# spirit-man/Planetary-LiDAR-Odometry

Hardware: AMD Instinct MI355X
Metric: IMLS-ICP scan-pairs/s (HDL-64 ~120k-pt scan vs 10-scan map, 20 ICP iterations) (higher is better)
Workload: dtype f64; 1 GPU; config B: HDL-64 scan vs 10-scan local map; a step = 4 independent scan pairs as 4 launch sequences in flight; queries=126189, map_points=1262664, solver=LS (trimmed, t=0.02), search_number=20, inputs=resident in HBM, fused_launch=True, launch_groups=4, parallelism=1 GPU, no process group

## Files before the change

### planetary-lidar-odometry_amd/csrc/project.hip

```cpp
#include <algorithm>
#include <cfloat>

#include "internal.h"
#include "geom.h"

#if defined(__has_builtin) && __has_builtin(__builtin_amdgcn_writelane)
__device__ __forceinline__ int imls_amdgcn_writelane(int v, int sel, int old) {
    return __builtin_amdgcn_writelane(v, sel, old);
}
#else
__device__ int imls_amdgcn_writelane(int v, int sel, int old) __asm("llvm.amdgcn.writelane");
#endif

namespace imlsgpu {
namespace {

constexpr double kInfD = __builtin_huge_val();
constexpr float kInfF = __builtin_huge_valf();
constexpr int kWaveBlock = 256;
typedef float kf4v __attribute__((ext_vector_type(4)));
typedef __attribute__((address_space(4))) const kf4v kconst_f4;
__device__ __forceinline__ int ld_const(const int* p) { return *(const __attribute__((address_space(4))) int*)p; }
__device__ __forceinline__ double ld_const(const double* p) { return *(const __attribute__((address_space(4))) double*)p; }
constexpr int kFallbackBlocks = 64;
// ... 66 lines not shown
    double dot = ns[0] * n0;
    dot = dot + ns[1] * n1;
    dot = dot + ns[2] * n2;
    double a = ns[0] * ns[0];
    a = a + ns[1] * ns[1];
    a = a + ns[2] * ns[2];
    double b = n0 * n0;
    b = b + n1 * n1;
    b = b + n2 * n2;
    const double s = sqrt(a) * sqrt(b);
    if (dot > (cthr + 2e-9) * s) return false;
    if (dot < (cthr - 2e-9) * s && dot >= -s * (1.0 - 1e-12)) return true;
    const double ca = dot / s;
    if (ca > cthr + 1e-9) return false;
    if (ca < cthr - 1e-9 && ca >= -1.0) return true;
    const double angle = acos(ca) * 180.0 / M_PI;
    return angle > thr;
}

template <int KL>
__device__ __forceinline__ void insert_top(float (&lk)[KL], int (&lp)[KL], float d, int pos) {
    bool c[KL];
#pragma unroll
    for (int k = 0; k < KL - 1; ++k) c[k] = d < lk[k];
    c[KL - 1] = true;
#pragma unroll
    for (int k = KL - 1; k >= 1; --k) {
        lp[k] = c[k - 1] ? lp[k - 1] : (c[k] ? pos : lp[k]);
        lk[k] = __builtin_amdgcn_fmed3f(lk[k - 1], d, lk[k]);
    }
    lp[0] = c[0] ? pos : lp[0];
    lk[0] = c[0] ? d : lk[0];
}

__device__ __forceinline__ float fmin_nn(float a, float b) { return a < b ? a : b; }

__device__ __forceinline__ void pin_loaded(const float4& v) { asm volatile("" ::"v"(v.x), "v"(v.y), "v"(v.z)); }

template <int KL>
__device__ __forceinline__ void insert_key(float (&lk)[KL], float d) {
#pragma unroll
    for (int k = KL - 1; k >= 1; --k) lk[k] = __builtin_amdgcn_fmed3f(lk[k - 1], d, lk[k]);
    lk[0] = fmin_nn(d, lk[0]);
}

template <int CAP, bool LAZY_D = false>
__device__ int finish_query(const float xf[3], const double ns[3], const double (&ld)[CAP], const int (&lpos)[CAP],
                            int first, int cnt, double d1, int p1, const TreeView& t, const KParams& kp, float yf[3],
                            float nf[3], int& kq, int qi) {
    if (p1 < 0) return IMLS_REJ_TOO_FAR;
    if (d1 > kp.h2) return IMLS_REJ_TOO_FAR;
    double nn[3];
    if (kp.tv) {
        const double4 v = t.tvn[qi];
        if (v.w == 0.0) return IMLS_REJ_NO_NORMAL;
        nn[0] = v.x; nn[1] = v.y; nn[2] = v.z;
    } else {
        if (!kp.get_normals) return IMLS_REJ_INVALID_NORMAL;
        const float4 n4 = t.mnr[p1];
        nn[0] = n4.x; nn[1] = n4.y; nn[2] = n4.z;
    }
    if (!(isfinite(nn[0]) && isfinite(nn[1]) && isfinite(nn[2]))) return IMLS_REJ_INVALID_NORMAL;
    if (kp.angle_on && angle_reject(ns, nn[0], nn[1], nn[2], kp.angle_thr_deg, kp.cos_thr)) return IMLS_REJ_NORMAL_CONSTRAINT;
    const double xd[3] = {xf[0], xf[1], xf[2]};
    unsigned long long acc = 0ull;
    int nacc = 0;
    constexpr int kChunk = 8;
#pragma unroll
    for (int j0 = 0; j0 < CAP; j0 += kChunk) {
        float4 qn[kChunk];
#pragma unroll
        for (int u = 0; u < kChunk; ++u) {
            const int j = j0 + u;
            const bool inl = j < CAP && j >= first && j < first + cnt;
            qn[u] = t.mnr[inl ? lpos[j < CAP ? j : 0] : p1];
        }
#pragma unroll
        for (int u = 0; u < kChunk; ++u) {
            const int j = j0 + u;
            const bool inl = j < CAP && j >= first && j < first + cnt;
            if (inl) {
                ++kq;
                bool ok = kp.get_normals && isfinite(qn[u].x) && isfinite(qn[u].y) && isfinite(qn[u].z);
                if (ok && kp.angle_on) ok = !angle_reject(ns, qn[u].x, qn[u].y, qn[u].z, kp.angle_thr_deg, kp.cos_thr);
                if (ok) { acc |= 1ull << j; ++nacc; }
            }
        }
    }
    if (nacc < 3) return IMLS_REJ_MLS_FAIL;
    const int target = first + nacc - 1;
    constexpr int kIChunk = IMLS_IMLS_CHUNK;
    float4 qp[kIChunk], qn[kIChunk];
    auto load_chunk = [&](int j0) {
#pragma unroll
        for (int u = 0; u < kIChunk; ++u) {
            const int j = j0 + u;
            const int pj = (j < CAP && (acc & (1ull << j))) ? lpos[j < CAP ? j : 0] : p1;
            qp[u] = t.mpt[pj];
            qn[u] = t.mnr[pj];
        }
    };
    auto pin_chunk = [&]() {
#pragma unroll
        for (int u = 0; u < kIChunk; ++u) {
            pin_loaded(qp[u]);
            pin_loaded(qn[u]);
        }
    };
    double dsel = 0.0;
    if (LAZY_D) {
        int ptg = p1;
#pragma unroll
        for (int j = 0; j < CAP; ++j) ptg = (j == target) ? lpos[j] : ptg;
        const float4 q = t.mpt[ptg];
        load_chunk(0);
        pin_loaded(q);
        pin_chunk();
        dsel = exact_d2(xd, q.x, q.y, q.z);
    } else {
#pragma unroll
        for (int j = 0; j < CAP; ++j) dsel = (j == target) ? ld[j] : dsel;
        load_chunk(0);
        pin_chunk();
    }
    const double hmax = sqrt(dsel) / 3;
    const double ih2 = 1.0 / (hmax * hmax);
    double wsum = 0.0, psum = 0.0;
#pragma unroll
    for (int j0 = 0; j0 < CAP; j0 += kIChunk) {
        if (j0 > 0) {
            if (!__ballot((acc >> j0) != 0ull)) break;
            if (!__ballot((acc >> j0) & ((1ull << kIChunk) - 1ull))) continue;
            load_chunk(j0);
            pin_chunk();
        }
#pragma unroll
        for (int u = 0; u < kIChunk; ++u) {
            const int j = j0 + u;
            if (j >= CAP) break;
            const bool a = (acc >> j) & 1ull;
            if (!__ballot(a)) continue;
            const double dx = xd[0] - (double)qp[u].x, dy = xd[1] - (double)qp[u].y, dz = xd[2] - (double)qp[u].z;
            double dn = dx * dx;
            dn = dn + dy * dy;
            dn = dn + dz * dz;
            const double w = exp(-dn * ih2);
            double pr = (w * dx) * (double)qn[u].x;
            pr = pr + (w * dy) * (double)qn[u].y;
            pr = pr + (w * dz) * (double)qn[u].z;
            wsum += a ? w : 0.0;
            psum += a ? pr : 0.0;
        }
    }
    const double height = psum / (wsum + 1e-5);
    if (isnan(height) || isinf(height)) return IMLS_REJ_NAN_INF_HEIGHT;
    yf[0] = (float)(xd[0] - height * nn[0]);
    yf[1] = (float)(xd[1] - height * nn[1]);
    yf[2] = (float)(xd[2] - height * nn[2]);
    nf[0] = (float)nn[0]; nf[1] = (float)nn[1]; nf[2] = (float)nn[2];
    return -1;
}

__device__ int finish_plane(const float xf[3], const double ns[3], int p1, const TreeView& t, const KParams& kp,
                            float yf[3], float nf[3]) {
    if (p1 < 0) return kp.proj ? IMLS_REJ_TOO_FAR : IMLS_REJ_NO_NORMAL;
    const float4 n4 = t.mnr[p1];
    const double nn[3] = {n4.x, n4.y, n4.z};
    if (!(isfinite(nn[0]) && isfinite(nn[1]) && isfinite(nn[2]))) return IMLS_REJ_INVALID_NORMAL;
    if (kp.angle_on && angle_reject(ns, nn[0], nn[1], nn[2], kp.angle_thr_deg, kp.cos_thr)) return IMLS_REJ_NORMAL_CONSTRAINT;
    const float4 q = t.mpt[p1];
    const double xd[3] = {xf[0], xf[1], xf[2]};
    const double v0 = xd[0] - (double)q.x, v1 = xd[1] - (double)q.y, v2 = xd[2] - (double)q.z;
    double pd = v0 * nn[0];
    pd = pd + v1 * nn[1];
    pd = pd + v2 * nn[2];
    yf[0] = (float)(xd[0] - pd * nn[0]);
    yf[1] = (float)(xd[1] - pd * nn[1]);
    yf[2] = (float)(xd[2] - pd * nn[2]);
    nf[0] = (float)nn[0]; nf[1] = (float)nn[1]; nf[2] = (float)nn[2];
    return -1;
}

__device__ __forceinline__ void plane_row(const float xf[3], const float yf[3], const float nf[3], double a[6], double& b) {
    const double s0 = xf[0], s1 = xf[1], s2 = xf[2];
    const double d0 = yf[0], d1 = yf[1], d2 = yf[2];
    const double n0 = nf[0], n1 = nf[1], n2 = nf[2];
    a[0] = n2 * s1 - n1 * s2;
    a[1] = n0 * s2 - n2 * s0;
    a[2] = n1 * s0 - n0 * s1;
    a[3] = n0; a[4] = n1; a[5] = n2;
    b = n0 * (d0 - s0);
    b = b + n1 * (d1 - s1);
    b = b + n2 * (d2 - s2);
}

template <int NT>
__device__ void block_normeq(const double a[6], double b, double one, double (*red)[kNormEq], double* out) {
    const int lane = threadIdx.x & 63, wv = threadIdx.x >> 6;
    int k = 0;
#pragma unroll
    for (int r = 0; r < 6; ++r) {
#pragma unroll
        for (int c = r; c < 6; ++c) {
            const double v = wave_total(a[r] * a[c]);
            if (lane == 63) red[wv][k] = v;
            ++k;
        }
    }
#pragma unroll
    for (int r = 0; r < 6; ++r) {
        const double v = wave_total(a[r] * b);
        if (lane == 63) red[wv][21 + r] = v;
    }
    {
        const double v = wave_total(one);
        if (lane == 63) red[wv][27] = v;
    }
    __syncthreads();
    if (threadIdx.x < kNormEq) {
        double s = 0.0;
#pragma unroll
        for (int w = 0; w < NT / 64; ++w) s += red[w][threadIdx.x];
        out[threadIdx.x] = s;
    }
    __syncthreads();
}

__device__ __forceinline__ void store_result(int i, int cat, const float xf[3], const float yf[3], const float nf[3],
                                             float4* cs, float4* cd, float4* cn) {
    cs[i] = make_float4(xf[0], xf[1], xf[2], cat == -1 ? 1.f : 0.f);
    if (cat == -1) {
        cd[i] = make_float4(yf[0], yf[1], yf[2], 0.f);
        cn[i] = make_float4(nf[0], nf[1], nf[2], 0.f);
    }
}

#ifdef IMLS_DEBUG_WAVE_TRACE
constexpr int kDbgWaves = 8192;
__device__ unsigned g_dbg_wave[kDbgWaves][16];
#endif


__device__ __forceinline__ bool verlet_skip(float4 xr, float nr, const float xf[3], float r2s, float& w_out,
                                            float& w_low) {
    const float dx = xf[0] - xr.x, dy = xf[1] - xr.y, dz = xf[2] - xr.z;
    const float D = sqrtf(__builtin_fmaf(dx, dx, __builtin_fmaf(dy, dy, dz * dz))) * (1.0f + 1e-6f) + 1e-6f;
    const float g = sqrtf(xr.w) * (1.0f - 1e-6f) - D;
    w_low = g > 0.f ? fminf(g * g, r2s) : -1.0f;
    if (!(g > 0.f) || !(nr < kInfF)) return false;
    const float u = sqrtf(nr) * (1.0f + 1e-6f) + D;
    const float w = fminf(g * g, r2s);
    w_out = w;
    return u * u * (1.0f + 1e-5f) < w;
}

template <int KL>
__device__ __forceinline__ float need_key(const float (&lk)[KL], float r2, int K) {
    const float r2f = r2 * (1.0f + 1e-6f);
    int cnt_r = 0;
    float dK = kInfF, d1 = kInfF;
#pragma unroll
    for (int j = 0; j < KL; ++j) {
        const bool in = lk[j] <= r2f;
        cnt_r += in ? 1 : 0;
        if (in && d1 == kInfF && lk[j] > 1e-15f) d1 = lk[j];
        if (j == K - 1) dK = lk[j];
    }
    return cnt_r >= K ? fmaxf(dK, d1) : (IMLS_UNDER_SKIN > 0 ? r2f : kInfF);
}

template <int KL>
struct IdKeys {
    static constexpr unsigned IDM = KL <= 32 ? 31u : 63u;
    static constexpr unsigned kSentinel = 0x7F7FFFFFu & ~IDM;
    __device__ static __forceinline__ float lo(float k) { return __uint_as_float(__float_as_uint(k) & ~IDM); }
    __device__ static __forceinline__ float hi(float k) { return __uint_as_float(__float_as_uint(k) | IDM); }
    __device__ static __forceinline__ unsigned id(float k) { return __float_as_uint(k) & IDM; }
    __device__ static __forceinline__ float make(float d, unsigned s) { return __uint_as_float((__float_as_uint(d) & ~IDM) | s); }
    __device__ static __forceinline__ float empty(unsigned s) { return __uint_as_float(kSentinel | s); }
    __device__ static __forceinline__ bool real(float k) { return (__float_as_uint(k) & ~IDM) < kSentinel; }
};

template <int KL>
__device__ __forceinline__ float need_key_ids(const float (&lk)[KL], float r2, int K) {
    using I = IdKeys<KL>;
    const float r2f = r2 * (1.0f + 1e-6f);
    int cnt_r = 0;
    float dK = kInfF, d1 = kInfF;
#pragma unroll
    for (int j = 0; j < KL; ++j) {
        const float up = I::hi(lk[j]);
        const bool in = I::real(lk[j]) && up <= r2f;
        cnt_r += in ? 1 : 0;
        if (in && d1 == kInfF && I::lo(lk[j]) > 1e-15f) d1 = up;
        if (j == K - 1) dK = up;
    }
    return cnt_r >= K ? fmaxf(dK, d1) : (IMLS_UNDER_SKIN > 0 ? r2f : kInfF);
}

#ifndef IMLS_KNN_WAVES
#define IMLS_KNN_WAVES 5
#endif
#define IMLS_KNN_ATTR __attribute__((amdgpu_waves_per_eu(KL <= 26 ? IMLS_KNN_WAVES : 2)))
template <int KL>
__device__ __forceinline__ void knn_wave_body(TreeView t, const float4* __restrict__ spt,
                                                         const unsigned* __restrict__ qperm, int N,
                                                         const double* __restrict__ pose,
                                                         const int* __restrict__ done, KParams kp,
                                                         const double* __restrict__ delta,
                                                         int* __restrict__ lists, float* __restrict__ wlist,
                                                         float4* __restrict__ xref, float* __restrict__ nref,
                                                         int use_prev, unsigned long long* __restrict__ nbr_stats,
                                                         int bx) {
    if (done && ld_const(done)) return;
    __shared__ int snode[kWaveBlock / 64][kWaveStack];
    __shared__ float4 sboxa[kWaveBlock / 64][kWaveStack];
    __shared__ float2 sboxb[kWaveBlock / 64][kWaveStack];
    __shared__ int spos[KL][kWaveBlock];
    const int tid = threadIdx.x, lane = tid & 63;
    int* const mypos = &spos[0][tid];
    using IK = IdKeys<KL>;
    const int wv = __builtin_amdgcn_readfirstlane(tid >> 6);
    const int qp = kp.packet;
    const int slot = (bx * (kWaveBlock / 64) + wv) * qp + lane;
    const bool active = lane < qp && slot < N;
    float xf[3] = {0.f, 0.f, 0.f};
    float w_prev = 0.f, n_prev = 0.f;
    float4 x_prev = make_float4(0.f, 0.f, 0.f, 0.f);
    if (active) {
        double ns[3];
        const int i = (int)qperm[slot];
        const float4 sp4 = spt[i];
        if (use_prev) {
            w_prev = wlist[slot];
            x_prev = xref[slot];
            n_prev = nref[slot];
        }
        transform_query(pose, sp4, make_float4(0.f, 0.f, 0.f, 0.f), 0, xf, ns);
    }
    float lk[KL];
#pragma unroll
    for (int j = 0; j < KL; ++j) lk[j] = IK::empty(j);
    if (use_prev) {
#pragma unroll
        for (int j = 0; j < KL; ++j) mypos[j * kWaveBlock] = -1;
    }
    auto thr_ = [&]() -> float { return IK::lo(lk[KL - 1]); };
    auto full_ = [&]() -> bool { return IK::real(lk[KL - 1]); };
    auto pos_ = [&](int s) -> int { return mypos[s * kWaveBlock]; };
    auto need_ = [&]() -> float { return need_key_ids<KL>(lk, (float)kp.r2, kp.K); };
    auto ins_ = [&](float d, int pos) {
        const unsigned s = IK::id(lk[KL - 1]);
        insert_key<KL>(lk, IK::make(d, s));
        mypos[s * kWaveBlock] = pos;
    };
    const float r2s = (float)(kp.r2 * kSearchR2) * kBoxSlack + 1e-30f;
    float bnd = active ? r2s : -1.0f;
    int P = t.P, B = t.B, M = t.M;
    asm volatile("" : "+s"(P), "+s"(B), "+s"(M));
#ifdef IMLS_DEBUG_WAVE_TRACE
    const long long dbg_t0 = wall_clock64();
#endif
    bool greedy = active && !use_prev;
    bool skip = false;
    float wskip = kInfF;
    if (active && use_prev) {
        double rf = 0.0;
#pragma unroll
        for (int r = 0; r < 3; ++r)
#pragma unroll
            for (int c = 0; c < 3; ++c) {
                const double e = ld_const(delta + r * 4 + c) - (r == c ? 1.0 : 0.0);
                rf += e * e;
            }
        const double d3 = ld_const(delta + 3), d7 = ld_const(delta + 7), d11 = ld_const(delta + 11);
        const float tn = (float)sqrt(d3 * d3 + d7 * d7 + d11 * d11);
        const float disp = tn + (float)sqrt(rf) * sqrtf(xf[0] * xf[0] + xf[1] * xf[1] + xf[2] * xf[2]);
        greedy = disp * disp > kReseed * w_prev;
    }
    float wlow = -1.0f;
    if (active && !greedy && kp.reuse) skip = verlet_skip(x_prev, n_prev, xf, r2s, wskip, wlow);
    if (active && !greedy && !skip) {
        int pj[KL];
#pragma unroll
        for (int j = 0; j < KL; ++j) pj[j] = lists[(size_t)j * N + slot];
        constexpr int kPCh = (KL + 1) / 2;
#pragma unroll
        for (int j0 = 0; j0 < KL; j0 += kPCh) {
            float4 q[kPCh];
#pragma unroll
            for (int u = 0; u < kPCh; ++u)
                if (j0 + u < KL) q[u] = t.mpt[max(pj[j0 + u], 0)];
#pragma unroll
            for (int u = 0; u < kPCh; ++u)
                if (j0 + u < KL) pin_loaded(q[u]);
#pragma unroll
            for (int u = 0; u < kPCh; ++u) {
                const int j = j0 + u;
                if (j >= KL) break;
                const float ex = q[u].x - xf[0], ey = q[u].y - xf[1], ez = q[u].z - xf[2];
                const float d32 = __builtin_fmaf(ex, ex, __builtin_fmaf(ey, ey, ez * ez));
                const bool keep = pj[j] >= 0 && d32 <= r2s;
                lk[j] = keep ? IK::make(d32, j) : IK::empty(j);
                mypos[j * kWaveBlock] = keep ? pj[j] : -1;
            }
        }
        bool swapped = true;
        while (swapped) {
            swapped = false;
#pragma unroll
            for (int par = 0; par < 2; ++par) {
#pragma unroll
                for (int j = par; j + 1 < KL; j += 2) {
                    const bool sw = lk[j + 1] < lk[j];
                    const float tk = lk[j];
                    lk[j] = sw ? lk[j + 1] : lk[j];
                    lk[j + 1] = sw ? tk : lk[j + 1];
                    swapped |= sw;
                }
            }
        }
        bnd = fmin_nn(r2s, thr_());
        if (kp.reuse && wlow > 0.f) {
            const float nk = need_();
            if (nk < kInfF && nk * (1.0f + 1e-5f) < wlow) { skip = true; wskip = wlow; }
        }
    }
#ifdef IMLS_DEBUG_WAVE_TRACE
    unsigned dbg_ev = 0, dbg_ins = 0;
    unsigned dbg_sparse = 0, dbg_bcast = 0, dbg_sparse_lanes = 0, dbg_listed_lv = 0;
    unsigned dbg_seed_steps = 0, dbg_seed_pts = 0;
#endif
    auto scan_leaf = [&](int leaf, unsigned long long want, bool listed, float4 mine) {
        const int base = leaf * B;
        const int cnt = min(B, M - base);
        unsigned long long inl = 0ull;
        auto listed_mask = [&]() {
#pragma unroll
            for (int k = 0; k < KL; ++k) {
                const unsigned rel = (unsigned)(pos_(k) - base);
                inl |= rel < 64u ? (1ull << rel) : 0ull;
            }
        };
        const bool sparse = __popcll(want) <= kSparseLanes;
        int bcast = __builtin_amdgcn_readfirstlane(!sparse);
        asm volatile("" : "+s"(bcast));
#ifdef IMLS_DEBUG_WAVE_TRACE
        if (sparse) { ++dbg_sparse; dbg_sparse_lanes += __popcll(want); } else { ++dbg_bcast; }
#endif
        if (sparse) {
            int nin = 0;
            bool have_inl = !listed;
            if (listed) {
#pragma unroll
                for (int k = 0; k < KL; ++k) nin += (unsigned)(pos_(k) - base) < (unsigned)cnt ? 1 : 0;
#ifdef IMLS_DEBUG_WAVE_TRACE
                dbg_listed_lv += (__ballot(nin > 0) & want) ? 1 : 0;
#endif
            }
            const float cb = fmin_nn(r2s, IK::hi(lk[KL - 1]));
            int cm_lo = 0, cm_hi = 0;
            const unsigned long long inleaf = cnt >= 64 ? ~0ull : (1ull << max(cnt, 0)) - 1ull;
            unsigned long long m = want;
            while (m) {
                const int q = __builtin_amdgcn_readfirstlane(__builtin_ctzll(m));
                m &= m - 1;
                const float qx = __int_as_float(__builtin_amdgcn_readlane(__float_as_int(xf[0]), q));
                const float qy = __int_as_float(__builtin_amdgcn_readlane(__float_as_int(xf[1]), q));
                const float qz = __int_as_float(__builtin_amdgcn_readlane(__float_as_int(xf[2]), q));
                const float qb = __int_as_float(__builtin_amdgcn_readlane(__float_as_int(cb), q));
                const float ex = mine.x - qx, ey = mine.y - qy, ez = mine.z - qz;
                const float d32 = __builtin_fmaf(ex, ex, __builtin_fmaf(ey, ey, ez * ez));
                unsigned long long pm = __ballot(d32 <= qb) & inleaf;
                if (!have_inl) {
                    const int nq = __builtin_amdgcn_readlane(nin, q);
                    if (__popcll(pm) > nq) {
                        listed_mask();
                        have_inl = true;
                    } else {
                        pm = 0ull;
                    }
                }
                if (pm) {
                    const unsigned long long inq =
                        ((unsigned long long)(unsigned)__builtin_amdgcn_readlane((int)(unsigned)(inl >> 32), q) << 32) |
                        (unsigned)__builtin_amdgcn_readlane((int)(unsigned)inl, q);
                    pm &= ~inq;
                }
                cm_lo = imls_amdgcn_writelane((int)(unsigned)pm, q, cm_lo);
                cm_hi = imls_amdgcn_writelane((int)(unsigned)(pm >> 32), q, cm_hi);
            }
            unsigned long long cm = ((unsigned long long)(unsigned)cm_hi << 32) | (unsigned)cm_lo;
            while (__ballot(cm != 0ull)) {
                const int jj = cm ? (int)__builtin_ctzll(cm) : 0;
                const float px = __shfl(mine.x, jj), py = __shfl(mine.y, jj), pz = __shfl(mine.z, jj);
                if (cm) {
                    cm &= cm - 1;
                    const float ex = px - xf[0], ey = py - xf[1], ez = pz - xf[2];
                    const float d32 = __builtin_fmaf(ex, ex, __builtin_fmaf(ey, ey, ez * ez));
                    if (d32 <= bnd && d32 < thr_()) {
#ifdef IMLS_DEBUG_WAVE_TRACE
                        ++dbg_ins;
#endif
                        ins_(d32, base + jj);
                        bnd = fmin_nn(r2s, thr_());
                    }
                }
#ifdef IMLS_DEBUG_WAVE_TRACE
                ++dbg_ev;
#endif
            }
        }
        if (bcast) {
            if (listed) listed_mask();
            const bool wants = (want >> lane) & 1ull;
#if IMLS_BCAST_SCALAR
            const kconst_f4* lp = (const kconst_f4*)t.mpt + base;
            kf4v g[kBcGroup];
#pragma unroll
            for (int u = 0; u < kBcGroup; ++u) g[u] = lp[min(u, cnt - 1)];
            for (int j0 = 0; j0 < cnt; j0 += kBcGroup) {
                kf4v nx[kBcGroup];
                const int jn = j0 + kBcGroup;
                if (jn + kBcGroup <= cnt) {
                    const kconst_f4* q = lp + jn;
#pragma unroll
                    for (int u = 0; u < kBcGroup; ++u) nx[u] = q[u];
                } else {
#pragma unroll
                    for (int u = 0; u < kBcGroup; ++u) nx[u] = lp[min(jn + u, cnt - 1)];
                }
                float d[kBcGroup];
                float dmin = kInfF;
#pragma unroll
                for (int u = 0; u < kBcGroup; ++u) {
                    const float ex = g[u].x - xf[0], ey = g[u].y - xf[1], ez = g[u].z - xf[2];
                    d[u] = __builtin_fmaf(ex, ex, __builtin_fmaf(ey, ey, ez * ez));
                    dmin = fminf(dmin, d[u]);
                }
                if (__ballot(wants && dmin <= bnd)) {
#pragma unroll
                    for (int u = 0; u < kBcGroup; ++u) {
                        const int j = j0 + u;
                        const bool ins = j < cnt && wants && d[u] <= bnd && d[u] < thr_() && !((inl >> j) & 1ull);
                        if (ins) {
                            ins_(d[u], base + j);
                            bnd = fmin_nn(r2s, thr_());
                        }
                    }
                }
#pragma unroll
                for (int u = 0; u < kBcGroup; ++u) g[u] = nx[u];
            }
#else
            for (int j = 0; j < cnt; ++j) {
                const float px = __int_as_float(__builtin_amdgcn_readlane(__float_as_int(mine.x), j));
                const float py = __int_as_float(__builtin_amdgcn_readlane(__float_as_int(mine.y), j));
                const float pz = __int_as_float(__builtin_amdgcn_readlane(__float_as_int(mine.z), j));
                const float ex = px - xf[0], ey = py - xf[1], ez = pz - xf[2];
                const float d32 = __builtin_fmaf(ex, ex, __builtin_fmaf(ey, ey, ez * ez));
                const bool ins = wants && d32 <= bnd && d32 < thr_() && !((inl >> j) & 1ull);
#ifdef IMLS_DEBUG_WAVE_TRACE
                const unsigned long long bi = __ballot(ins);
                dbg_ev += bi ? 1 : 0;
                dbg_ins += __popcll(bi);
#endif
                if (ins) {
                    ins_(d32, base + j);
                    bnd = fmin_nn(r2s, thr_());
                }
            }
#endif
        }
    };
    const unsigned long long gmask = __ballot(greedy);
    static_assert(KL * kWaveBlock * 4 >= kSeedTab * 8, "seed table fits the slot array");
    unsigned long long* const skey = reinterpret_cast<unsigned long long*>(&spos[0][0]);
    const int S = use_prev ? t.L : (t.L + kSeedTab - 1) / kSeedTab;
    const int ntab = S > 0 ? (t.L + S - 1) / S : 0;
    if (!use_prev) {
        for (int k = threadIdx.x; k < ntab; k += kWaveBlock) skey[k] = t.lkeys[(size_t)k * S];
        __syncthreads();
    }
    int seed_leaf = 0;
    if (greedy) {
        const unsigned long long qk = morton48(xf[0], xf[1], xf[2], t.qparams);
        int j = 0, jh = ntab - 1;
        while (j < jh) {
            const int mid = (j + jh + 1) >> 1;
            if (skey[mid] <= qk) j = mid;
            else jh = mid - 1;
        }
        int l = j * S, h = min(t.L, (j + 1) * S) - 1;
        while (l < h) {
            const int mid = (l + h + 1) >> 1;
            if (t.lkeys[mid] <= qk) l = mid;
            else h = mid - 1;
        }
        seed_leaf = l;
    }
    if (!use_prev) {
        __syncthreads();
#pragma unroll
        for (int j = 0; j < KL; ++j) mypos[j * kWaveBlock] = -1;
    }
    if (greedy) {
        const int l = seed_leaf;
        const int p0s = max(0, l - kSeedHalf) * B;
        const int pend = min(M, (min(t.L - 1, l + kSeedHalf) + 1) * B);
        float4 qs[kSeedChunk];
#pragma unroll
        for (int k = 0; k < kSeedChunk; ++k) qs[k] = t.mpt[min(p0s + k, pend - 1)];
        for (int p0 = p0s; p0 < pend; p0 += kSeedChunk) {
            float4 nx[kSeedChunk];
#pragma unroll
            for (int k = 0; k < kSeedChunk; ++k) nx[k] = t.mpt[min(p0 + kSeedChunk + k, pend - 1)];
#pragma unroll
            for (int k = 0; k < kSeedChunk; ++k) {
                const float ex = qs[k].x - xf[0], ey = qs[k].y - xf[1], ez = qs[k].z - xf[2];
                const float d32 = __builtin_fmaf(ex, ex, __builtin_fmaf(ey, ey, ez * ez));
#ifdef IMLS_DEBUG_WAVE_TRACE
                dbg_seed_steps += __ballot(p0 + k < pend && d32 <= bnd && d32 < thr_()) ? 1 : 0;
                ++dbg_seed_pts;
#endif
                if (p0 + k < pend && d32 <= bnd && d32 < thr_()) {
                    ins_(d32, p0 + k);
                    bnd = fmin_nn(r2s, thr_());
                }
            }
#pragma unroll
            for (int k = 0; k < kSeedChunk; ++k) qs[k] = nx[k];
        }
    }
    unsigned n_inner = 0, n_leaf = 0;
#ifdef IMLS_DEBUG_WAVE_TRACE
    const long long dbg_t1 = wall_clock64();
#endif
    if (skip) bnd = -1.0f;
    int node = 1, sp = 0;
#if IMLS_LEAF_PREFETCH
    int pf_leaf = -1;
    float4 pf = make_float4(0.f, 0.f, 0.f, 0.f);
#endif
    unsigned long long em = __ballot(active && !skip);
    const unsigned long long skipped = __ballot(skip);
    if (nbr_stats && lane == 0 && skipped) atomicAdd(&nbr_stats[kStatSkipped], (unsigned long long)__popcll(skipped));
    while (em) {
        int pop = 1;
        int at_leaf = __builtin_amdgcn_readfirstlane(node >= P);
        asm volatile("" : "+s"(at_leaf));
        if (node < P) {
            ++n_inner;
            const int lev = 31 - __builtin_clz(node);
            const int sw = min(kWide, t.levels - lev);
            const int nk = 1 << sw, nrec = nk >> 1;
            const int unode = __builtin_amdgcn_readfirstlane(node);
            const kconst_f4* rec = (const kconst_f4*)t.nodes + 3 * ((size_t)unode << (sw - 1));
            float2 cb0 = make_float2(0.f, 0.f), cb1 = cb0, cb2 = cb0;
            if (lane < nk) {
                const float2* cp = reinterpret_cast<const float2*>(t.nodes + 3 * ((size_t)unode << (sw - 1))) + 3 * lane;
                cb0 = cp[0]; cb1 = cp[1]; cb2 = cp[2];
            }
            float4 R[3 * (kWideMax / 2)];
#pragma unroll
            for (int k = 0; k < 3 * (kWideMax / 2); ++k) {
                const kf4v v = rec[min(k, 3 * nrec - 1)];
                R[k] = make_float4(v.x, v.y, v.z, v.w);
            }
            const float bs = bnd * kBoxSlack;
            unsigned long long m[kWideMax];
            int best = -1;
            float bd = kInfF;
#pragma unroll
            for (int k = 0; k < kWideMax; ++k) {
                const float4 a = R[3 * (k >> 1)], b = R[3 * (k >> 1) + 1], c = R[3 * (k >> 1) + 2];
                const float d = (k & 1) ? box_d2(xf, b.z, b.w, c.x, c.y, c.z, c.w) : box_d2(xf, a.x, a.y, a.z, a.w, b.x, b.y);
                const bool w = k < nk && d <= bs;
                m[k] = __ballot(w);
                if (w && d < bd) { bd = d; best = k; }
            }
            int cstar = -1, vbest = 0;
            unsigned long long mstar = 0ull;
#pragma unroll
            for (int k = 0; k < kWideMax; ++k) {
                const int v = __popcll(__ballot(best == k));
                if (m[k] && (cstar < 0 || v > vbest)) { cstar = k; vbest = v; mstar = m[k]; }
            }
            unsigned wm = 0u;
#pragma unroll
            for (int k = 0; k < kWideMax; ++k) wm |= m[k] ? (1u << k) : 0u;
            const unsigned pm = cstar >= 0 ? wm & ~(1u << cstar) : 0u;
            if (lane < kWideMax && ((pm >> lane) & 1u)) {
                const int pos = sp + __popc(pm >> (lane + 1));
                snode[wv][pos] = (node << sw) + lane;
                sboxa[wv][pos] = make_float4(cb0.x, cb0.y, cb1.x, cb1.y);
                sboxb[wv][pos] = cb2;
            }
            if (cstar >= 0) {
                sp += __popc(pm);
                em = mstar;
                node = (node << sw) + cstar;
                pop = 0;
            }
        }
        if (at_leaf) {
            ++n_leaf;
            const int leaf = node - P;
            float4 mine = make_float4(0.f, 0.f, 0.f, 0.f);
#if IMLS_LEAF_PREFETCH
            if (leaf == pf_leaf) mine = pf;
            else if (lane < min(B, M - leaf * B)) mine = t.mpt[leaf * B + lane];
            pf_leaf = -1;
            if (sp > 0) {
                const int nn = __builtin_amdgcn_readfirstlane(snode[wv][sp - 1]);
                if (nn >= P) {
                    pf_leaf = nn - P;
                    pf = make_float4(0.f, 0.f, 0.f, 0.f);
                    if (lane < min(B, M - pf_leaf * B)) pf = t.mpt[pf_leaf * B + lane];
                }
            }
#else
            if ((!IMLS_BCAST_SCALAR || __popcll(em) <= kSparseLanes) && lane < min(B, M - leaf * B))
                mine = t.mpt[leaf * B + lane];
#endif
            scan_leaf(leaf, em, use_prev || gmask, mine);
        }
        asm volatile("" : "+s"(pop));
        if (pop) {
            em = 0ull;
            while (sp > 0 && !em) {
                --sp;
                const float4 b0 = sboxa[wv][sp];
                const float2 b1 = sboxb[wv][sp];
                const float d = box_d2(xf, b0.x, b0.y, b0.z, b0.w, b1.x, b1.y);
                em = __ballot(d <= bnd * kBoxSlack);
            }
            if (em) node = snode[wv][sp];
        }
    }
    if (active && skip) wlist[slot] = wskip;
    if (active && !skip) {
#pragma unroll
        for (int j = 0; j < KL; ++j) lists[(size_t)j * N + slot] = pos_(IK::id(lk[j]));
        const bool full = full_();
        const float wk = full ? thr_() : kInfF;
        wlist[slot] = wk;
        xref[slot] = make_float4(xf[0], xf[1], xf[2], full ? wk : r2s);
        nref[slot] = need_();
    }
#ifdef IMLS_DEBUG_WAVE_TRACE
    if (nbr_stats && lane == 0) {
        atomicAdd(&nbr_stats[6], (unsigned long long)dbg_ev);
        atomicAdd(&nbr_stats[7], (unsigned long long)dbg_ins);
    }
    if (nbr_stats && lane == 0) {
        const long long dbg_t2 = wall_clock64();
        atomicAdd(&nbr_stats[8], (unsigned long long)(dbg_t1 - dbg_t0));
        atomicMax(&nbr_stats[9], (unsigned long long)(dbg_t1 - dbg_t0));
        atomicAdd(&nbr_stats[10], (unsigned long long)(dbg_t2 - dbg_t1));
        atomicMax(&nbr_stats[11], (unsigned long long)(dbg_t2 - dbg_t1));
        atomicAdd(&nbr_stats[12], (unsigned long long)n_leaf);
        atomicMax(&nbr_stats[13], (unsigned long long)n_leaf);
        atomicMax(&nbr_stats[14], (unsigned long long)dbg_ev);
        atomicAdd(&nbr_stats[15], (unsigned long long)__popcll(__ballot(greedy)));
    }
    {
        const unsigned long long gl = __ballot(greedy), wi = __ballot(active && !full_()),
                                 w1 = __ballot(active && full_() && thr_() > 1.0f);
        float wmax = active && full_() ? thr_() : 0.f;
        for (int o = 1; o < 64; o <<= 1) wmax = fmaxf(wmax, __shfl_xor(wmax, o));
        if (lane == 0) {
            const int w = bx * (kWaveBlock / 64) + wv;
            if (w < kDbgWaves) {
                unsigned* r = g_dbg_wave[w];
                r[0] = (unsigned)(dbg_t1 - dbg_t0); r[1] = (unsigned)(wall_clock64() - dbg_t1);
                r[2] = n_leaf; r[3] = n_inner; r[4] = dbg_ev; r[5] = dbg_sparse; r[6] = dbg_bcast;
                r[7] = __popcll(gl); r[8] = __popcll(wi); r[9] = __popcll(w1); r[10] = __float_as_uint(wmax);
                r[11] = dbg_sparse_lanes; r[12] = dbg_listed_lv; r[13] = dbg_ins;
                r[14] = dbg_seed_steps; r[15] = __builtin_amdgcn_readfirstlane(dbg_seed_pts);
            }
        }
    }
#endif
    if (nbr_stats && lane == 0) {
        atomicAdd(&nbr_stats[2], (unsigned long long)n_leaf);
        atomicAdd(&nbr_stats[3], (unsigned long long)n_inner);
        atomicAdd(&nbr_stats[4], 1ull);
    }
}

template <int KL>
__device__ __forceinline__ void finish_q_core(TreeView t, const float4* __restrict__ spt, const float4* __restrict__ snr,
                                              int i, int slot, const double* __restrict__ pose, const KParams& kp,
                                              int pos, float W, float4* __restrict__ cs, float4* __restrict__ cd,
                                              float4* __restrict__ cn, imls_iter_trace* __restrict__ tr,
                                              unsigned long long* __restrict__ nbr_stats, int* stk_n, float* stk_d);
struct QFinishArgs {
    const float4* snr;
    float4 *cs, *cd, *cn;
    imls_iter_trace* tr;
};
template <int KL, bool FUSED = false>
__device__ __forceinline__ void knn_qwave_body(TreeView t, const float4* __restrict__ spt,
                                                          const unsigned* __restrict__ qperm, int N,
                                                          const double* __restrict__ pose,
                                                          const int* __restrict__ done, KParams kp,
                                                          const double* __restrict__ delta,
                                                          int* __restrict__ lists, float* __restrict__ wlist,
                                                          float4* __restrict__ xref, float* __restrict__ nref,
                                                          int use_prev, unsigned long long* __restrict__ nbr_stats,
                                                          int bx, const QFinishArgs& fa = QFinishArgs{}) {
    static_assert(KL <= 64, "one list entry per lane");
    if (done && ld_const(done)) return;
    __shared__ int snode[kWaveBlock / 64][kWaveStack];
    __shared__ float sdist[kWaveBlock / 64][kWaveStack];
    __shared__ int fnode[kWaveBlock / 64][kFStack];
    __shared__ float fdist[kWaveBlock / 64][kFStack];
    const int lane = threadIdx.x & 63;
    const int wv = __builtin_amdgcn_readfirstlane(threadIdx.x >> 6);
    const int slot = __builtin_amdgcn_readfirstlane(bx * (kWaveBlock / 64) + wv);
    if (slot >= N) return;
#ifdef IMLS_DEBUG_WAVE_TRACE
    const long long dbg_q0 = wall_clock64();
#endif
    float xf[3];
    {
        double ns[3];
        transform_query(pose, spt[qperm[slot]], make_float4(0.f, 0.f, 0.f, 0.f), 0, xf, ns);
    }
    float lkey = kInfF;
    int lpos = -1;
    const float r2s = (float)(kp.r2 * kSearchR2) * kBoxSlack + 1e-30f;
    const float h2s = (float)kp.h2 * kBoxSlack + 1e-30f;
    bool hmode = false;
    float bnd = r2s;
    const int P = t.P, B = t.B, M = t.M;
    auto insert = [&](float c, int cp) {
        const unsigned long long before = __ballot(lane < KL && (lkey < c || (lkey == c && lpos < cp)));
        const int at = __popcll(before);
        const float uk = __shfl_up(lkey, 1, 64);
        const int up = __shfl_up(lpos, 1, 64);
        if (lane > at && lane < KL) { lkey = uk; lpos = up; }
        if (lane == at) { lkey = c; lpos = cp; }
        bnd = fminf(hmode ? h2s : r2s, __int_as_float(__builtin_amdgcn_readlane(__float_as_int(lkey), KL - 1)));
    };
    auto worst = [&]() { return __int_as_float(__builtin_amdgcn_readlane(__float_as_int(lkey), KL - 1)); };
    int seed_lo = 0, seed_hi = -1, seed_leaf = -1;
    bool greedy = !use_prev;
    bool skip = false;
    float wskip = kInfF;
    if (use_prev) {
        double rf = 0.0;
#pragma unroll
        for (int r = 0; r < 3; ++r)
#pragma unroll
            for (int c = 0; c < 3; ++c) {
                const double e = ld_const(delta + r * 4 + c) - (r == c ? 1.0 : 0.0);
                rf += e * e;
            }
        const double d3 = ld_const(delta + 3), d7 = ld_const(delta + 7), d11 = ld_const(delta + 11);
        const float tn = (float)sqrt(d3 * d3 + d7 * d7 + d11 * d11);
        const float disp = tn + (float)sqrt(rf) * sqrtf(xf[0] * xf[0] + xf[1] * xf[1] + xf[2] * xf[2]);
        greedy = disp * disp > kReseed * wlist[slot];
    }
    float wlow = -1.0f;
    if (!greedy && kp.reuse) skip = verlet_skip(xref[slot], nref[slot], xf, r2s, wskip, wlow);
    if (skip) {
    } else if (!greedy) {
        const int pos = lane < KL ? lists[(size_t)lane * N + slot] : -1;
        float d = kInfF;
        if (pos >= 0) {
            const float4 q = t.mpt[pos];
            const float ex = q.x - xf[0], ey = q.y - xf[1], ez = q.z - xf[2];
            d = __builtin_fmaf(ex, ex, __builtin_fmaf(ey, ey, ez * ez));
        }
        const bool in = pos >= 0 && d <= bnd;
        float sk = in ? d : kInfF;
        int sp = in ? pos : -1;
        constexpr int W = KL <= 32 ? 32 : 64;
#pragma unroll
        for (int size = 2; size <= W; size <<= 1) {
#pragma unroll
            for (int stride = size >> 1; stride > 0; stride >>= 1) {
                const float ok = __shfl_xor(sk, stride, 64);
                const int op = __shfl_xor(sp, stride, 64);
                const bool asc = (lane & size) == 0, low = (lane & stride) == 0;
                const bool other_less = ok < sk || (ok == sk && op < sp);
                const bool other_more = sk < ok || (sk == ok && sp < op);
                if (asc == low ? other_less : other_more) { sk = ok; sp = op; }
            }
        }
        if (lane < KL) { lkey = sk; lpos = sp; }
        bnd = fminf(r2s, worst());
    } else {
        const unsigned long long qk = morton48(xf[0], xf[1], xf[2], t.qparams);
        int lo = 0, hi = t.L - 1;
        while (lo < hi) {
            const int mid = (lo + hi + 1) >> 1;
            if (t.lkeys[mid] <= qk) lo = mid;
            else hi = mid - 1;
        }
        seed_lo = max(0, lo - kSeedHalf);
        seed_hi = min(t.L - 1, lo + kSeedHalf);
        seed_leaf = lo;
        for (int leaf = seed_lo; leaf <= seed_hi; ++leaf) {
            const int base = leaf * B, cnt = min(B, M - base);
            float d = kInfF;
            if (lane < cnt) {
                const float4 q = t.mpt[base + lane];
                const float ex = q.x - xf[0], ey = q.y - xf[1], ez = q.z - xf[2];
                d = __builtin_fmaf(ex, ex, __builtin_fmaf(ey, ey, ez * ez));
            }
            unsigned long long m = __ballot(lane < cnt && d <= bnd);
            while (m) {
                const int j = __builtin_ctzll(m);
                m &= m - 1;
                const float c = __int_as_float(__builtin_amdgcn_readlane(__float_as_int(d), j));
                if (c <= bnd && c < worst()) insert(c, base + j);
            }
        }
    }
    unsigned n_inner = 0, n_leaf = 0;
    if (nbr_stats && lane == 0 && skip) atomicAdd(&nbr_stats[kStatSkipped], 1ull);
    auto nearest = [&]() { return __int_as_float(__builtin_amdgcn_readfirstlane(__float_as_int(lkey))); };
    if (!skip && kp.matcher == IMLS_MATCH_IMLS && !(nearest() <= h2s)) {
        hmode = true;
        bnd = fminf(bnd, h2s);
    }
    for (int pass = 0; pass < 2; ++pass) {
    int node = 0, sp = 0;
    if (!skip) {
        const int p0 = __builtin_amdgcn_readfirstlane(lpos);
        const int sl = greedy ? seed_leaf : (p0 >= 0 ? p0 / B : -1);
        node = 1;
        if (sl >= 0) {
            const int ln = P + sl;
            float d = kInfF;
            int sn = 0;
            if (lane < t.levels) {
                sn = (ln >> lane) ^ 1;
                const float4* rec = t.nodes + 3 * (size_t)(sn >> 1);
                const float4 a = rec[0], b = rec[1], c = rec[2];
                d = (sn & 1) ? box_d2(xf, b.z, b.w, c.x, c.y, c.z, c.w) : box_d2(xf, a.x, a.y, a.z, a.w, b.x, b.y);
            }
            const unsigned long long want = __ballot(lane < t.levels && d <= bnd * kBoxSlack);
            if ((want >> lane) & 1ull) {
                const int at = __popcll(want >> (lane + 1));
                snode[wv][at] = sn;
                sdist[wv][at] = d;
            }
            sp = __popcll(want);
            node = ln;
        }
    }
    if (node) {
        if (lane < sp) { fnode[wv][lane] = snode[wv][lane]; fdist[wv][lane] = sdist[wv][lane]; }
        if (lane == 0) { fnode[wv][sp] = node; fdist[wv][sp] = 0.0f; }
        int fsp = sp + 1;
        const int ppl = (B + 7) >> 3;
#ifdef IMLS_DEBUG_WAVE_TRACE
        int dbg_steps = 0;
#endif
        while (fsp > 0) {
#ifdef IMLS_DEBUG_WAVE_TRACE
            if (++dbg_steps > 20000 || fsp > kFStack) {
                if (lane == 0)
                    printf("frontier stuck: slot %d pass %d steps %d fsp %d sp0 %d node0 %d bnd %g P %d levels %d B %d M %d\n",
                           slot, pass, dbg_steps, fsp, sp, node, (double)bnd, P, t.levels, B, M);
                break;
            }
#endif
            const int lim = fsp > kFBatchMax ? 1 : 8;
            const int idx = fsp - 1 - lane;
            int en = 0;
            float ed = kInfF;
            if (idx >= 0) { en = fnode[wv][idx]; ed = fdist[wv][idx]; }
            const unsigned long long vm = __ballot(idx >= 0 && ed <= bnd * kBoxSlack);
            unsigned long long rem = vm, taken = 0;
            int gsrc[8];
            int ng = 0;
#pragma unroll
            for (int g = 0; g < 8; ++g) {
                gsrc[g] = 0;
                if (g < lim && rem) {
                    const int b = __builtin_ctzll(rem);
                    gsrc[g] = b;
                    taken |= 1ull << b;
                    rem &= rem - 1;
                    ++ng;
                }
            }
            fsp -= (ng == lim) ? (64 - __builtin_clzll(taken)) : min(fsp, 64);
            if (!ng) continue;
            const int g = lane >> 3, gl = lane & 7;
            int src = gsrc[0];
#pragma unroll
            for (int k = 1; k < 8; ++k) src = g == k ? gsrc[k] : src;
            const int gnode = __shfl(en, src, 64);
            const bool gact = g < ng;
            const bool ginner = gact && gnode < P, gleaf = gact && gnode >= P;
            n_inner += __popcll(__ballot(ginner && gl == 0));
            n_leaf += __popcll(__ballot(gleaf && gl == 0));
            float cdist = kInfF;
            int child = 0;
            int sw = 0;
            if (ginner) sw = min(kWide, t.levels - (31 - __builtin_clz(gnode)));
            const bool gbox = ginner && gl < (1 << sw);
            const float4* rec = t.nodes + 3 * (gbox ? (((size_t)gnode << (sw - 1)) + (gl >> 1)) : (size_t)1);
            const float4 ra = rec[0], rb = rec[1], rc = rec[2];
            int lbase = 0, lcnt = 0;
            if (gleaf) {
                const int leaf = gnode - P;
                if (leaf < seed_lo || leaf > seed_hi) {
                    lbase = leaf * B;
                    lcnt = min(B, M - lbase);
                }
            }
            float4 lq[8];
#pragma unroll
            for (int k = 0; k < 8; ++k) {
                const int j = gl + 8 * k;
                lq[k] = t.mpt[(k < ppl && j < lcnt) ? lbase + j : 0];
            }
            pin_loaded(ra);
            pin_loaded(rb);
            pin_loaded(rc);
#pragma unroll
            for (int k = 0; k < 8; ++k) pin_loaded(lq[k]);
            if (gbox) {
                cdist = (gl & 1) ? box_d2(xf, rb.z, rb.w, rc.x, rc.y, rc.z, rc.w) : box_d2(xf, ra.x, ra.y, ra.z, ra.w, rb.x, rb.y);
                child = (gnode << sw) + gl;
            }
            float pd[8];
#pragma unroll
            for (int k = 0; k < 8; ++k) {
                const int j = gl + 8 * k;
                const float ex = lq[k].x - xf[0], ey = lq[k].y - xf[1], ez = lq[k].z - xf[2];
                const float d = __builtin_fmaf(ex, ex, __builtin_fmaf(ey, ey, ez * ez));
                pd[k] = (k < ppl && j < lcnt) ? d : kInfF;
            }
#pragma unroll
            for (int k = 0; k < 8; ++k) {
                if (k >= ppl) break;
                unsigned long long m = __ballot(pd[k] <= bnd && pd[k] < worst());
                while (m) {
                    const int j = __builtin_ctzll(m);
                    m &= m - 1;
                    const float cd = __int_as_float(__builtin_amdgcn_readlane(__float_as_int(pd[k]), j));
                    const int cp = __builtin_amdgcn_readlane(lbase + gl + 8 * k, j);
                    if (cd <= bnd && cd < worst() && !__ballot(lane < KL && lpos == cp)) insert(cd, cp);
                }
            }
            const unsigned long long want = __ballot(child != 0 && cdist <= bnd * kBoxSlack);
            if ((want >> lane) & 1ull) {
                const int at = fsp + (lane == 63 ? 0 : __popcll(want >> (lane + 1)));
                fnode[wv][at] = child;
                fdist[wv][at] = cdist;
            }
            fsp += __popcll(want);
        }
    }
    if (!hmode) break;
    if (!(nearest() <= h2s)) {
        lkey = kInfF;
        lpos = -1;
        break;
    }
    hmode = false;
    bnd = fminf(r2s, worst());
    }
    if (skip) {
        if (lane == 0) wlist[slot] = wskip;
    } else {
        if (lane < KL) lists[(size_t)lane * N + slot] = lpos;
        const bool lpos_any = __ballot(lane < KL && lpos >= 0) != 0ull;
        float lkr[KL];
#pragma unroll
        for (int k = 0; k < KL; ++k) lkr[k] = __int_as_float(__builtin_amdgcn_readlane(__float_as_int(lkey), k));
        const float nk = lpos_any ? need_key<KL>(lkr, (float)kp.r2, kp.K) : kInfF;
        if (lane == 0) {
            const float wk = worst();
// ... 1489 lines not shown
```

Measured before the change: 471.9 scan-pairs/s.

## Use DPP wave reductions for child vote and hoist listed-mask out of sparse loop

```diff
diff --git a/planetary-lidar-odometry_amd/csrc/project.hip b/planetary-lidar-odometry_amd/csrc/project.hip
--- a/planetary-lidar-odometry_amd/csrc/project.hip
+++ b/planetary-lidar-odometry_amd/csrc/project.hip
@@ -392,6 +392,23 @@
 #define IMLS_KNN_WAVES 5
 #endif
 #define IMLS_KNN_ATTR __attribute__((amdgpu_waves_per_eu(KL <= 26 ? IMLS_KNN_WAVES : 2)))
+constexpr int kDppShr1 = 0x111, kDppShr2 = 0x112, kDppShr4 = 0x114, kDppShr8 = 0x118;
+constexpr int kDppBcast15 = 0x142, kDppBcast31 = 0x143;
+template <int CTRL, int ROWS = 0xf>
+__device__ __forceinline__ int dpp_i(int old, int v) { return __builtin_amdgcn_update_dpp(old, v, CTRL, ROWS, 0xf, false); }
+struct RedOr { static constexpr int id = 0; __device__ static __forceinline__ int op(int a, int b) { return a | b; } };
+struct RedAdd { static constexpr int id = 0; __device__ static __forceinline__ int op(int a, int b) { return a + b; } };
+template <class R>
+__device__ __forceinline__ int wave_reduce(int v) {
+    v = R::op(v, dpp_i<kDppShr1>(R::id, v));
+    v = R::op(v, dpp_i<kDppShr2>(R::id, v));
+    v = R::op(v, dpp_i<kDppShr4>(R::id, v));
+    v = R::op(v, dpp_i<kDppShr8>(R::id, v));
+    v = R::op(v, dpp_i<kDppBcast15, 0xa>(R::id, v));
+    return R::op(v, dpp_i<kDppBcast31, 0xc>(R::id, v));
+}
+__device__ __forceinline__ int wave_last(int v) { return __builtin_amdgcn_readlane(v, 63); }
+
 template <int KL>
 __device__ __forceinline__ void knn_wave_body(TreeView t, const float4* __restrict__ spt,
                                                          const unsigned* __restrict__ qperm, int N,
@@ -519,6 +536,7 @@
 #ifdef IMLS_DEBUG_WAVE_TRACE
     unsigned dbg_ev = 0, dbg_ins = 0;
     unsigned dbg_sparse = 0, dbg_bcast = 0, dbg_sparse_lanes = 0, dbg_listed_lv = 0;
+    unsigned dbg_mask_lv = 0;
     unsigned dbg_seed_steps = 0, dbg_seed_pts = 0;
 #endif
     auto scan_leaf = [&](int leaf, unsigned long long want, bool listed, float4 mine) {
@@ -540,7 +558,6 @@
 #endif
         if (sparse) {
             int nin = 0;
-            bool have_inl = !listed;
             if (listed) {
 #pragma unroll
                 for (int k = 0; k < KL; ++k) nin += (unsigned)(pos_(k) - base) < (unsigned)cnt ? 1 : 0;
@@ -554,47 +571,42 @@
             unsigned long long m = want;
             while (m) {
                 const int q = __builtin_amdgcn_readfirstlane(__builtin_ctzll(m));
-                m &= m - 1;
+                m &= ~(1ull << q);
                 const float qx = __int_as_float(__builtin_amdgcn_readlane(__float_as_int(xf[0]), q));
                 const float qy = __int_as_float(__builtin_amdgcn_readlane(__float_as_int(xf[1]), q));
                 const float qz = __int_as_float(__builtin_amdgcn_readlane(__float_as_int(xf[2]), q));
                 const float qb = __int_as_float(__builtin_amdgcn_readlane(__float_as_int(cb), q));
                 const float ex = mine.x - qx, ey = mine.y - qy, ez = mine.z - qz;
                 const float d32 = __builtin_fmaf(ex, ex, __builtin_fmaf(ey, ey, ez * ez));
-                unsigned long long pm = __ballot(d32 <= qb) & inleaf;
-                if (!have_inl) {
-                    const int nq = __builtin_amdgcn_readlane(nin, q);
-                    if (__popcll(pm) > nq) {
-                        listed_mask();
-                        have_inl = true;
-                    } else {
-                        pm = 0ull;
-                    }
-                }
-                if (pm) {
-                    const unsigned long long inq =
-                        ((unsigned long long)(unsigned)__builtin_amdgcn_readlane((int)(unsigned)(inl >> 32), q) << 32) |
-                        (unsigned)__builtin_amdgcn_readlane((int)(unsigned)inl, q);
-                    pm &= ~inq;
-                }
+                const unsigned long long pm = __ballot(d32 <= qb) & inleaf;
                 cm_lo = imls_amdgcn_writelane((int)(unsigned)pm, q, cm_lo);
                 cm_hi = imls_amdgcn_writelane((int)(unsigned)(pm >> 32), q, cm_hi);
             }
             unsigned long long cm = ((unsigned long long)(unsigned)cm_hi << 32) | (unsigned)cm_lo;
+            if (listed) {
+                if (__ballot(__popcll(cm) > nin)) {
+#ifdef IMLS_DEBUG_WAVE_TRACE
+                    ++dbg_mask_lv;
+#endif
+                    listed_mask();
+                    cm &= ~inl;
+                } else {
+                    cm = 0ull;
+                }
+            }
             while (__ballot(cm != 0ull)) {
-                const int jj = cm ? (int)__builtin_ctzll(cm) : 0;
+                const bool has = cm != 0ull;
+                const int jj = has ? (int)__builtin_ctzll(cm) : 0;
                 const float px = __shfl(mine.x, jj), py = __shfl(mine.y, jj), pz = __shfl(mine.z, jj);
-                if (cm) {
-                    cm &= cm - 1;
-                    const float ex = px - xf[0], ey = py - xf[1], ez = pz - xf[2];
-                    const float d32 = __builtin_fmaf(ex, ex, __builtin_fmaf(ey, ey, ez * ez));
-                    if (d32 <= bnd && d32 < thr_()) {
+                cm &= cm - 1ull;
+                const float ex = px - xf[0], ey = py - xf[1], ez = pz - xf[2];
+                const float d32 = __builtin_fmaf(ex, ex, __builtin_fmaf(ey, ey, ez * ez));
+                if (has & (d32 <= bnd) & (d32 < thr_())) {
 #ifdef IMLS_DEBUG_WAVE_TRACE
-                        ++dbg_ins;
-#endif
-                        ins_(d32, base + jj);
-                        bnd = fmin_nn(r2s, thr_());
-                    }
+                    ++dbg_ins;
+#endif
+                    ins_(d32, base + jj);
+                    bnd = fmin_nn(r2s, thr_());
                 }
 #ifdef IMLS_DEBUG_WAVE_TRACE
                 ++dbg_ev;
@@ -752,13 +764,14 @@
                 cb0 = cp[0]; cb1 = cp[1]; cb2 = cp[2];
             }
             float4 R[3 * (kWideMax / 2)];
+            const unsigned lastb = (unsigned)(3 * nrec - 1) * 16u;
 #pragma unroll
             for (int k = 0; k < 3 * (kWideMax / 2); ++k) {
-                const kf4v v = rec[min(k, 3 * nrec - 1)];
+                const kf4v v = *(const kconst_f4*)((const __attribute__((address_space(4))) char*)rec + min((unsigned)k * 16u, lastb));
                 R[k] = make_float4(v.x, v.y, v.z, v.w);
             }
             const float bs = bnd * kBoxSlack;
-            unsigned long long m[kWideMax];
+            unsigned wbits = 0u;
             int best = -1;
             float bd = kInfF;
 #pragma unroll
@@ -766,19 +779,20 @@
                 const float4 a = R[3 * (k >> 1)], b = R[3 * (k >> 1) + 1], c = R[3 * (k >> 1) + 2];
                 const float d = (k & 1) ? box_d2(xf, b.z, b.w, c.x, c.y, c.z, c.w) : box_d2(xf, a.x, a.y, a.z, a.w, b.x, b.y);
                 const bool w = k < nk && d <= bs;
-                m[k] = __ballot(w);
+                wbits |= w ? (1u << k) : 0u;
                 if (w && d < bd) { bd = d; best = k; }
             }
-            int cstar = -1, vbest = 0;
-            unsigned long long mstar = 0ull;
-#pragma unroll
-            for (int k = 0; k < kWideMax; ++k) {
-                const int v = __popcll(__ballot(best == k));
-                if (m[k] && (cstar < 0 || v > vbest)) { cstar = k; vbest = v; mstar = m[k]; }
-            }
-            unsigned wm = 0u;
-#pragma unroll
-            for (int k = 0; k < kWideMax; ++k) wm |= m[k] ? (1u << k) : 0u;
+            const unsigned hot = best < 0 ? 0u : 1u << ((best & 3) * 8);
+            const unsigned wm = (unsigned)wave_last(wave_reduce<RedOr>((int)wbits));
+            const unsigned vlo = (unsigned)wave_last(wave_reduce<RedAdd>((int)(best < 4 ? hot : 0u)));
+            const unsigned vhi = (unsigned)wave_last(wave_reduce<RedAdd>((int)(best < 4 ? 0u : hot)));
+            const unsigned cnt = (unsigned)((((unsigned long long)vhi << 32) | vlo) >> ((lane & 7) * 8)) & 0xffu;
+            unsigned key = (wm >> (lane & 7)) & 1u ? ((cnt << 3) | (unsigned)(7 - (lane & 7))) + 1u : 0u;
+            key = max(key, (unsigned)dpp_i<kDppShr1>(0, (int)key));
+            key = max(key, (unsigned)dpp_i<kDppShr2>(0, (int)key));
+            key = max(key, (unsigned)dpp_i<kDppShr4>(0, (int)key));
+            const unsigned kmax = (unsigned)__builtin_amdgcn_readlane((int)key, 7);
+            const int cstar = kmax == 0u ? -1 : 7 - (int)((kmax - 1u) & 7u);
             const unsigned pm = cstar >= 0 ? wm & ~(1u << cstar) : 0u;
             if (lane < kWideMax && ((pm >> lane) & 1u)) {
                 const int pos = sp + __popc(pm >> (lane + 1));
@@ -788,7 +802,7 @@
             }
             if (cstar >= 0) {
                 sp += __popc(pm);
-                em = mstar;
+                em = __ballot((wbits >> cstar) & 1u);
                 node = (node << sw) + cstar;
                 pop = 0;
             }
@@ -866,7 +880,7 @@
                 r[0] = (unsigned)(dbg_t1 - dbg_t0); r[1] = (unsigned)(wall_clock64() - dbg_t1);
                 r[2] = n_leaf; r[3] = n_inner; r[4] = dbg_ev; r[5] = dbg_sparse; r[6] = dbg_bcast;
                 r[7] = __popcll(gl); r[8] = __popcll(wi); r[9] = __popcll(w1); r[10] = __float_as_uint(wmax);
-                r[11] = dbg_sparse_lanes; r[12] = dbg_listed_lv; r[13] = dbg_ins;
+                r[11] = dbg_sparse_lanes; r[12] = dbg_listed_lv | (dbg_mask_lv << 16); r[13] = dbg_ins;
                 r[14] = dbg_seed_steps; r[15] = __builtin_amdgcn_readfirstlane(dbg_seed_pts);
             }
         }
```

Result: faster. 500.2 scan-pairs/s, median of 6 (+6.0%).
